# LiuZhu-CV/PAIF

Hardware: AMD Instinct MI355X
Metric: fused image-pairs/sec at 480x640 bs=8 per GPU (fusion-net forward) (higher is better)
Workload: dtype f16 (IEEE fp16 maps and conv weights, one fp16 MFMA per product, f32 accumulate; stems, guided filter and the last map fp32)

## Files before the change

include/paif_hip.h:

```cpp
#ifndef PAIF_HIP_H
#define PAIF_HIP_H

#include <stddef.h>
#include <stdint.h>

#ifdef __cplusplus
extern "C" {
#endif

#define PAIF_ABI_VERSION 1
#define PAIF_EINVAL (-1)
#define PAIF_ENOSUP (-2)

typedef void* paif_stream_t;

int paif_version(void);
const char* paif_last_error(void);
int paif_device_cus(void);


int paif_rgb2ycrcb_fwd(const float* rgb, float* ycc, int B, int H, int W, paif_stream_t stream);

int paif_ycrcb2rgb_fwd(const float* ycc, float* rgb, int B, int H, int W, paif_stream_t stream);

// ... 62 lines not shown
  float* cpool;
} paif_conv_desc;
#define PAIF_ST_F32 0
#define PAIF_ST_BF16 1
#define PAIF_ST_F32_BF16 2
#define PAIF_ST_F16 3
#define PAIF_ST_F16_F32 4
#define PAIF_CONV_F32 0
#define PAIF_CONV_BF16X3 1
#define PAIF_CONV_BF16 2
#define PAIF_CONV_F16 4
#define PAIF_CONV_F16X2 5
#define PAIF_CONV_F16X3 6
#define PAIF_CONV_BF16X6 3

int paif_dwconv_fwd_bf16(const float* x, const float* w, float* out, int k, int dil, int in_relu, int B, int H, int W,
                         paif_stream_t stream);
int paif_channel_pool2_fwd_bf16(const float* ir, const float* vis, float* comp, int B, int H, int W, paif_stream_t stream);
int paif_spa_blend_fwd_bf16(const float* comp, const float* w, const float* ir, const float* vis, float* agg, int B, int H, int W,
                            paif_stream_t stream);
int paif_eca_finish_fwd_bf16(const float* o, const float* r, const float* pool_partial, const float* w1d, int k,
                             const float* prelu, float* gate, float* out, int B, int H, int W, paif_stream_t stream);
int paif_tail_fwd_bf16(const float* x, const float* w, const float* prelu, float* fused, int B, int H, int W, paif_stream_t stream);
int paif_add_fwd_bf16(const float* a, const float* b, float* out, size_t n, paif_stream_t stream);
int paif_cast_storage_fwd(const float* src, float* dst, size_t n, int mode, paif_stream_t stream);
int paif_dwconv_fwd_f16(const float* x, const float* w, float* out, int k, int dil, int in_relu, int B, int H, int W,
                        paif_stream_t stream);
int paif_channel_pool2_fwd_f16(const float* ir, const float* vis, float* comp, int B, int H, int W, paif_stream_t stream);
int paif_spa_blend_fwd_f16(const float* comp, const float* w, const float* ir, const float* vis, float* agg, int B, int H, int W,
                           paif_stream_t stream);
int paif_eca_finish_fwd_f16(const float* o, const float* r, const float* pool_partial, const float* w1d, int k,
                            const float* prelu, float* gate, float* out, int B, int H, int W, paif_stream_t stream);
int paif_tail_fwd_f16(const float* x, const float* w, const float* prelu, float* fused, int B, int H, int W, paif_stream_t stream);
int paif_add_fwd_f16(const float* a, const float* b, float* out, size_t n, paif_stream_t stream);

int paif_conv2d_blocks(int B, int H, int W);
int paif_conv2d_fwd(const paif_conv_desc* d, int B, int H, int W, paif_stream_t stream);
int paif_conv2d_can_cpool(const paif_conv_desc* d, int B, int H, int W);
int paif_channel_pool1_fwd(const float* x, float* comp_off, int B, int H, int W, paif_stream_t stream);
int paif_channel_pool1_fwd_bf16(const float* x, float* comp_off, int B, int H, int W, paif_stream_t stream);
int paif_channel_pool1_fwd_f16(const float* x, float* comp_off, int B, int H, int W, paif_stream_t stream);
int paif_conv2d_is_persistent(const paif_conv_desc* d, int B, int H, int W);
int paif_conv2d_kernel_name(const paif_conv_desc* d, int B, int H, int W, char* buf, int buflen);
size_t paif_conv_wpk_floats(int nsrc, int cin, int kh);
int paif_pack_conv_weight(const float* w, float* wpk, int cout, int nsrc, int cin, int kh, paif_stream_t stream);
int paif_pack_conv_weight_bf16x3(const float* w, float* wpk, int cout, int nsrc, int kh, paif_stream_t stream);
int paif_pack_conv_weight_f16x2(const float* w, float* wpk, int cout, int nsrc, int kh, paif_stream_t stream);
int paif_pack_conv_weight_bf16x6(const float* w, float* wpk, int cout, int nsrc, int kh, paif_stream_t stream);
int paif_compose_dw_pw_weight(const float* dw, const float* pw, float* out, int cout, int cin, int kh, paif_stream_t stream);
int paif_compose_pw_conv_weight(const float* pw, const float* w, float* out, int cout, int cmid, int cin, int kh, paif_stream_t stream);

size_t paif_rdb_fused_wpk_floats(void);
int paif_rdb_fused_pack(const float* w1, const float* w2, const float* w3, float* wpk, int f16, paif_stream_t stream);
int paif_rdb_fused_fwd(const float* x, const float* wpk, const float* prelu, float alpha, const float* res0, const float* res1, float* out,
                       float* cpool, int f16, int reverse_tiles, int B, int H, int W, paif_stream_t stream);

int paif_stem_out_pack_floats(void);
int paif_stem_out_pack(const float* w1, const float* w2, float* wpk, paif_stream_t stream);
int paif_stem_out_fwd_bf16(const float* x, const float* wpk, const float* prelu, float* fused, int B, int H, int W, paif_stream_t stream);
int paif_stem_out_fwd_f32(const float* x, const float* wpk, const float* prelu, float* fused, int B, int H, int W, paif_stream_t stream);
int paif_stem_out_fwd_guard(const float* x, int f32in, const float* wpk, const float* prelu, float* fused, unsigned* flag, int B, int H, int W,
                            paif_stream_t stream);
int paif_pack_decomp1x1_weight_bf16x6(const float* w, float* wpk, paif_stream_t stream);
int paif_pack_decomp1x1_weight_bf16x3(const float* w, float* wpk, paif_stream_t stream);
int paif_pack_decomp1x1_hf_weight_f16x2(const float* w, float* wpk, paif_stream_t stream);
int paif_pack_decomp1x1_weight(const float* w, float* wpk, paif_stream_t stream);
// ... 260 lines not shown
```

paif_amd/_lib.py:

```python
import ctypes
import os
from ctypes import POINTER, Structure, c_char_p, c_float, c_int, c_size_t, c_ulonglong, c_void_p

HERE = os.path.dirname(os.path.abspath(__file__))
LIB_PATH = os.environ.get("PAIF_LIB") or os.path.join(HERE, "lib", "libpaif_hip.so")

F = c_void_p


class ConvDesc(Structure):

    _fields_ = [
        ("src", F * 3), ("nsrc", c_int), ("cin", c_int), ("wpk", F), ("kh", c_int), ("dil", c_int),
        ("in_act", c_int), ("in_prelu", F), ("scale", F), ("shift", F), ("act", c_int), ("prelu", F),
        ("alpha", c_float), ("res", F * 3), ("out", F), ("cout", c_int), ("pool_partial", F),
        ("precision", c_int), ("aux_out", F), ("in_aux", F), ("in_scale", F), ("in_alpha", c_float), ("epi_aux", F),
        ("epi_dact", c_int), ("reverse_tiles", c_int), ("storage", c_int), ("cpool", F),
    ]


SIGNATURES = {
    "paif_version": (c_int, []),
    "paif_last_error": (c_char_p, []),
    "paif_device_cus": (c_int, []),
# ... 81 lines not shown
    "paif_layernorm_fwd": (c_int, [F, F, F, F, c_int, c_int, c_float, F]),
    "paif_im2col_fwd": (c_int, [F, F, c_int, c_int, c_int, c_int, c_int, c_int, c_int, c_int, F]),
    "paif_pack_conv_gemm_weight": (c_int, [F, F, c_int, c_int, c_int, c_int, F]),
    "paif_dwconv3_bias_gelu_fwd": (c_int, [F, F, F, F, c_int, c_int, c_int, c_int, F]),
    "paif_sr_attention_fwd": (c_int, [F, F, F, F, c_int, c_int, c_int, c_int, c_int, F]),
    "paif_sr_attention_bf16x3_fwd": (c_int, [F, F, F, F, c_int, c_int, c_int, c_int, c_int, F]),
    "paif_sr_attention_split_fwd": (c_int, [F, F, F, F, c_int, c_int, c_int, c_int, c_int, c_int, F]),
    "paif_resize_bilinear_into_fwd": (c_int, [F, F, c_int, c_int, c_int, c_int, c_int, c_int, c_int, c_int, F]),
    "paif_nhwc_to_nchw_fwd": (c_int, [F, F, c_int, c_int, c_int, F]),
    "paif_nchw_to_nhwc_fwd": (c_int, [F, F, c_int, c_int, c_int, F]),
    "paif_nchw_to_nhwc_pad_fwd": (c_int, [F, F, c_int, c_int, c_int, c_int, F]),
    "paif_gemm_masked_fwd": (c_int, [F, c_int, F, F, F, F, F, c_int, F, c_int, F, c_int, c_int, c_int, c_int, c_int, F]),
    "paif_transpose_pad_fwd": (c_int, [F, F, c_int, c_int, c_int, F]),
    "paif_layernorm_bwd_input": (c_int, [F, F, F, F, F, c_int, c_int, c_float, F]),
    "paif_dwconv3_bias_gelu_bwd_input": (c_int, [F, F, F, F, F, F, c_int, c_int, c_int, c_int, F]),
    "paif_col2im_fwd": (c_int, [F, F, c_int, c_int, c_int, c_int, c_int, c_int, c_int, c_int, F]),
    "paif_resize_bilinear_adjoint_fwd": (c_int, [F, F, c_int, c_int, c_int, c_int, c_int, c_int, c_int, c_int, F]),
    "paif_sr_attention_bwd_chunks": (c_int, [c_int, c_int, c_int]),
    "paif_sr_attention_bwd_input": (c_int, [F, F, F, F, F, F, F, F, F, c_int, c_int, c_int, c_int, c_int, F]),
    "paif_sr_attention_bwd_input_p": (c_int, [F, F, F, F, F, F, F, F, F, c_int, c_int, c_int, c_int, c_int, c_int, F]),
    "paif_upsample_ce_blocks": (c_int, [c_int, c_int, c_int]),
    "paif_upsample_ce_fwd": (c_int, [F, F, F, F, c_int, c_int, c_int, c_int, c_int, c_int, c_int, F]),
    "paif_dwconv_fwd_bf16": (c_int, [F, F, F, c_int, c_int, c_int, c_int, c_int, c_int, F]),
    "paif_channel_pool2_fwd_bf16": (c_int, [F, F, F, c_int, c_int, c_int, F]),
    "paif_spa_blend_fwd_bf16": (c_int, [F, F, F, F, F, c_int, c_int, c_int, F]),
    "paif_eca_finish_fwd_bf16": (c_int, [F, F, F, F, c_int, F, F, F, c_int, c_int, c_int, F]),
    "paif_tail_fwd_bf16": (c_int, [F, F, F, F, c_int, c_int, c_int, F]),
    "paif_add_fwd_bf16": (c_int, [F, F, F, c_size_t, F]),
    "paif_dwconv_fwd_f16": (c_int, [F, F, F, c_int, c_int, c_int, c_int, c_int, c_int, F]),
    "paif_channel_pool2_fwd_f16": (c_int, [F, F, F, c_int, c_int, c_int, F]),
    "paif_spa_blend_fwd_f16": (c_int, [F, F, F, F, F, c_int, c_int, c_int, F]),
    "paif_eca_finish_fwd_f16": (c_int, [F, F, F, F, c_int, F, F, F, c_int, c_int, c_int, F]),
    "paif_tail_fwd_f16": (c_int, [F, F, F, F, c_int, c_int, c_int, F]),
    "paif_add_fwd_f16": (c_int, [F, F, F, c_size_t, F]),
    "paif_cast_storage_fwd": (c_int, [F, F, c_size_t, c_int, F]),
    "paif_attack_loss_blocks": (c_int, [c_int, c_int, c_int]),
    "paif_attack_loss_fwd": (c_int, [F, F, F, F, c_int, c_float, c_float, c_int, c_int, c_int, c_int, c_int, c_int, c_int, F]),
    "paif_attack_loss_bwd": (c_int, [F, F, F, F, c_int, c_float, c_float, c_float, c_int, c_int, c_int, c_int, c_int, c_int, c_int, c_int, F]),
    "paif_conv_weight_dgrad": (c_int, [F, F, c_int, c_int, c_int, c_int, c_int, F]),
    "paif_fold_decomp1x1_weight": (c_int, [F, F, F]),
    "paif_tail_bwd_input": (c_int, [F, F, F, F, F, F, c_int, c_int, c_int, F]),
    "paif_stem_bwd_input": (c_int, [F, F, F, F, F, c_int, c_int, c_int, F]),
    "paif_dwconv_bwd_input": (c_int, [F, F, F, F, F, c_int, c_int, c_int, c_int, c_int, F]),
    "paif_eca_bwd_blocks": (c_int, [c_int, c_int]),
    "paif_eca_bwd_input": (c_int, [F, F, F, F, F, c_int, F, F, F, F, F, c_int, c_int, c_int, F]),
    "paif_spa_blend_bwd_input": (c_int, [F, F, F, F, F, F, F, F, F, F, c_int, c_int, c_int, F]),
    "paif_guided_filter_bwd_input": (c_int, [F, F, F, F, c_float, c_float, F, F, F, F, F, F, c_int, c_int, c_int, F]),
    "paif_guided_filter_bwd_input_mc": (c_int, [F, F, F, F, F, F, F, F, F, F, c_int, c_int, c_int, F]),
    "paif_upsample_argmax_fwd": (c_int, [F, F, c_int, c_int, c_int, c_int, c_int, c_int, F]),
    "paif_confusion_matrix_accum": (c_int, [F, F, F, c_size_t, c_int, F]),
    "paif_spa1_fwd": (c_int, [F, F, F, c_int, F, F, F, F, F, c_int, c_int, c_int, F]),
    "paif_spa1_bwd_input": (c_int, [F, F, F, F, F, c_int, F, F, F, F, c_int, c_int, c_int, F]),
    "paif_glue_bwd_blocks": (c_int, [c_int, c_int, c_int]),
    "paif_glue_bwd_input": (c_int, [F, F, F, F, F, F, F, F, c_int, c_int, c_int, F]),
    "paif_plane_minmax_blocks": (c_int, [c_size_t]),
    "paif_plane_clamp_minmax_fwd": (c_int, [F, F, F, F, c_size_t, F]),
    "paif_plane_clamp_minmax_bwd_input": (c_int, [F, F, F, F, F, c_size_t, F]),
    "paif_channel_sum_chunks_fwd": (c_int, [F, F, c_int, c_int, c_int, c_int, F]),
    "paif_rgb2ycrcb_bwd_input": (c_int, [F, F, F, c_int, c_int, c_int, F]),
    "paif_pgd_step": (c_int, [F, F, F, c_float, c_float, c_size_t, F]),
    "paif_axpy": (c_int, [F, F, c_float, c_size_t, F]),
    "paif_upsample_ce_bwd": (c_int, [F, F, F, F, c_int, c_int, c_int, c_int, c_int, c_int, c_int, c_int, F]),
    "paif_head_sum_fwd": (c_int, [F, F, F, F, POINTER(c_int), F, F, F, c_int, c_int, F]),
    "paif_relu_mask_scale_fwd": (c_int, [F, F, F, F, c_size_t, c_int, F]),
    "paif_u8_to_planes_fwd": (c_int, [F, F, c_int, c_int, c_int, F]),
    "paif_u8_to_i64_fwd": (c_int, [F, F, c_size_t, F]),
# ... 71 lines not shown
```

paif_amd/csrc/fusion_kernels.hip:

```cpp
#include <stdarg.h>

#include "paif_common.h"

namespace paif {
static thread_local char g_err[256] = "";
void set_error(const char* fmt, ...) {
  va_list ap;
  va_start(ap, fmt);
  vsnprintf(g_err, sizeof(g_err), fmt, ap);
  va_end(ap);
}
}

namespace {

constexpr int MAXGRID = 256 * 8;

inline int grid_for(size_t work_items, int per_block) {
  size_t g = (work_items + per_block - 1) / per_block;
  if (g > (size_t)MAXGRID) g = MAXGRID;
  if (g < 1) g = 1;
  return (int)g;
}

__global__ void rgb2ycrcb_kernel(const float* __restrict__ rgb, float* __restrict__ ycc, int B, size_t HW) {
  const size_t total = (size_t)B * HW;
  for (size_t i = (size_t)blockIdx.x * blockDim.x + threadIdx.x; i < total; i += (size_t)gridDim.x * blockDim.x) {
    const size_t b = i / HW, px = i - b * HW;
    const float* s = rgb + b * 3 * HW + px;
    const float R = s[0], G = s[HW], Bl = s[2 * HW];
    const float Y = __fadd_rn(__fadd_rn(__fmul_rn(0.299f, R), __fmul_rn(0.587f, G)), __fmul_rn(0.114f, Bl));
    const float Cr = __fadd_rn(__fmul_rn(__fsub_rn(R, Y), 0.713f), 0.5f);
    const float Cb = __fadd_rn(__fmul_rn(__fsub_rn(Bl, Y), 0.564f), 0.5f);
    float* d = ycc + b * 3 * HW + px;
// ... 857 lines not shown
}
int paif_channel_pool1_fwd(const float* x, float* comp_off, int B, int H, int W, paif_stream_t stream) { return channel_pool1_launch(x, comp_off, B, H, W, 0, stream); }
int paif_channel_pool1_fwd_bf16(const float* x, float* comp_off, int B, int H, int W, paif_stream_t stream) { return channel_pool1_launch(x, comp_off, B, H, W, 1, stream); }
int paif_channel_pool1_fwd_f16(const float* x, float* comp_off, int B, int H, int W, paif_stream_t stream) { return channel_pool1_launch(x, comp_off, B, H, W, 2, stream); }

int paif_dwconv_fwd_bf16(const float* x, const float* w, float* out, int k, int dil, int in_relu, int B, int H, int W, paif_stream_t stream) {
  return dwconv16<1>(x, w, out, k, dil, in_relu, B, H, W, stream);
}
int paif_dwconv_fwd_f16(const float* x, const float* w, float* out, int k, int dil, int in_relu, int B, int H, int W, paif_stream_t stream) {
  return dwconv16<2>(x, w, out, k, dil, in_relu, B, H, W, stream);
}
int paif_channel_pool2_fwd_bf16(const float* ir, const float* vis, float* comp, int B, int H, int W, paif_stream_t stream) {
  return channel_pool2_16<1>(ir, vis, comp, B, H, W, stream);
}
int paif_channel_pool2_fwd_f16(const float* ir, const float* vis, float* comp, int B, int H, int W, paif_stream_t stream) {
  return channel_pool2_16<2>(ir, vis, comp, B, H, W, stream);
}
int paif_spa_blend_fwd_bf16(const float* comp, const float* w, const float* ir, const float* vis, float* agg, int B, int H, int W,
                            paif_stream_t stream) {
  return spa_blend16<1>(comp, w, ir, vis, agg, B, H, W, stream);
}
int paif_spa_blend_fwd_f16(const float* comp, const float* w, const float* ir, const float* vis, float* agg, int B, int H, int W,
                           paif_stream_t stream) {
  return spa_blend16<2>(comp, w, ir, vis, agg, B, H, W, stream);
}
int paif_eca_finish_fwd_bf16(const float* o, const float* r, const float* pool_partial, const float* w1d, int k, const float* prelu,
                             float* gate, float* out, int B, int H, int W, paif_stream_t stream) {
  return eca_finish16<1>(o, r, pool_partial, w1d, k, prelu, gate, out, B, H, W, stream);
}
int paif_eca_finish_fwd_f16(const float* o, const float* r, const float* pool_partial, const float* w1d, int k, const float* prelu,
                            float* gate, float* out, int B, int H, int W, paif_stream_t stream) {
  return eca_finish16<2>(o, r, pool_partial, w1d, k, prelu, gate, out, B, H, W, stream);
}
int paif_tail_fwd_bf16(const float* x, const float* w, const float* prelu, float* fused, int B, int H, int W, paif_stream_t stream) {
  return tail16<1>(x, w, prelu, fused, B, H, W, stream);
}
int paif_tail_fwd_f16(const float* x, const float* w, const float* prelu, float* fused, int B, int H, int W, paif_stream_t stream) {
  return tail16<2>(x, w, prelu, fused, B, H, W, stream);
}
int paif_add_fwd_bf16(const float* a, const float* b, float* out, size_t n, paif_stream_t stream) { return add16<1>(a, b, out, n, stream); }
int paif_add_fwd_f16(const float* a, const float* b, float* out, size_t n, paif_stream_t stream) { return add16<2>(a, b, out, n, stream); }

int paif_cast_storage_fwd(const float* src, float* dst, size_t n, int mode, paif_stream_t stream) {
  PAIF_REQUIRE(src && dst && n % 4 == 0, PAIF_EINVAL, "cast_storage: null pointer or n %% 4 != 0");
  PAIF_REQUIRE(mode >= 0 && mode <= 3, PAIF_EINVAL, "cast_storage: mode=%d", mode);
  if (n == 0) return 0;
  const dim3 g(grid_for(n / 4, 256)), blk(256);
  hipStream_t st = paif::as_stream(stream);
  switch (mode) {
    case 0: hipLaunchKernelGGL((cast_storage_kernel<1, 0>), g, blk, 0, st, src, dst, n / 4); break;
    case 1: hipLaunchKernelGGL((cast_storage_kernel<0, 1>), g, blk, 0, st, src, dst, n / 4); break;
    case 2: hipLaunchKernelGGL((cast_storage_kernel<0, 2>), g, blk, 0, st, src, dst, n / 4); break;
    default: hipLaunchKernelGGL((cast_storage_kernel<2, 0>), g, blk, 0, st, src, dst, n / 4); break;
  }
  PAIF_LAUNCH_CHECK("cast_storage");
  return 0;
}

int paif_minmax_blocks(int B, int H, int W) {
  const size_t total = (size_t)B * H * W;
  return (int)((total + MM_BLOCK_PIX - 1) / MM_BLOCK_PIX);
}

int paif_recompose_clamp_fwd(const float* fused, const float* ycc, float* rgb_out, float* minmax_partial, int B, int H,
                             int W, paif_stream_t stream) {
  PAIF_REQUIRE(fused && ycc && rgb_out && minmax_partial && B > 0 && H > 0 && W > 0, PAIF_EINVAL,
// ... 21 lines not shown
```

paif_amd/operations_m.py:

```python
import torch
import torch.nn as nn

from . import ops


class _NeverCalled:
    def forward(self, *a, **k):
        raise RuntimeError("%s is a parameter holder; the HIP path must be used" % type(self).__name__)


class Conv2dParams(_NeverCalled, nn.Conv2d):
    pass


class Conv1dParams(_NeverCalled, nn.Conv1d):
    pass


class BatchNormParams(_NeverCalled, nn.BatchNorm2d):
    pass


class PReLUParams(_NeverCalled, nn.PReLU):
    pass
# ... 435 lines not shown

class eca_layer(nn.Module):

    def __init__(self, channel, c_out, stride, k_size=3):
        super().__init__()
        self.k_size = k_size
        self.conv = Conv1dParams(1, 1, kernel_size=k_size, padding=(k_size - 1) // 2, bias=False)

    def forward(self, x):
        ops.require_no_grad(x)
        if x.shape[1] != 32:
            raise NotImplementedError("eca_layer: the HIP kernels are built for the 32-channel maps of the search space")
        with torch.no_grad():
            return ops.to_nchw_view(ops.eca_layer_fwd(ops.to_nhwc(x), self.conv.weight, self.k_size))


class ECABasicBlock(_HipOp):

    def __init__(self, inplanes, planes, kernel=3, dilation=1, stride=1, reduction=64, with_norm=False):
        super().__init__()
        if with_norm:
            raise NotImplementedError("ECABasicBlock(with_norm=True) is never constructed by the reference")
        self.with_norm = with_norm
        self.k = kernel
        self.conv1 = conv3x3(inplanes, planes, stride)
        self.conv2 = BasicConv(inplanes, inplanes, kernel, relu=False)
        self.se = eca_layer(planes, planes, stride, k_size=kernel)
        self.relu = PReLUParams()

    def forward_nhwc(self, x, res=(), tape=None):
        a = self.relu.weight
        w1 = self._packs.get("w1", [self.conv1.weight], lambda: ops.pack_conv_weight(self.conv1.weight, 1, 32, 3))
        r = ops.conv2d([x], w1, 3, 1)
        o, partial = ops.conv2d([r], self.conv2.wpk(1, 32), self.k, 1, in_act=ops.ACT_PRELU, in_prelu=a, pool=True)
        if tape is None:
            out = ops.eca_finish(o, r, partial, self.se.conv.weight, self.k, a)
        else:
            out, u, gate = ops.eca_finish(o, r, partial, self.se.conv.weight, self.k, a, save=True)
            tape.append(dict(r=r, o=o, u=u, gate=gate, x=x, pool=partial) if ops.taping_wgrad() else dict(r=r, o=o, u=u, gate=gate))
        return self._add_res(out, res)

    bwd_takes_res = True

    def backward_nhwc(self, g, t, wgrad=False, res=()):
        a = self.relu.weight
        if not wgrad:
            d_o, d_r = ops.eca_bwd(g, t["u"], t["o"], t["gate"], self.se.conv.weight, self.k, a)
            d_r = ops.conv2d([d_o], self._dgrad_w("c2", self.conv2.conv.weight), self.k, 1, epi_dact=1, epi_aux=t["r"], prelu=a, res=(d_r,))
            return ops.conv2d([d_r], self._dgrad_w("c1", self.conv1.weight), 3, 1, res=tuple(res))
        B, H, W, _ = g.shape
        ds = ops.grad_of(a)
        if ds is not None:
            ops.prelu_bwd(g, t["u"], a, ds)
        d_o, d_r, dgate = ops.eca_bwd(g, t["u"], t["o"], t["gate"], self.se.conv.weight, self.k, a, want_partial=True)
        g1d = ops.grad_of(self.se.conv.weight)
        if g1d is not None:
            ops.eca_wgrad(t["pool"], dgate, t["gate"], self.k, g1d, B, H, W)
        gw2 = ops.grad_of(self.conv2.conv.weight)
        if gw2 is not None:
            ops.conv2d_wgrad([ops.affine_act_res(t["r"], None, None, ops.ACT_PRELU, a)], d_o, self.k, 1, out=gw2)
        tt = ops.conv2d([d_o], self._dgrad_w("c2", self.conv2.conv.weight), self.k, 1)
        d_r = ops.prelu_bwd(tt, t["r"], a, ds, add=d_r, want_dx=True)
        gw1 = ops.grad_of(self.conv1.weight)
        if gw1 is not None:
            ops.conv2d_wgrad([t["x"]], d_r, 3, 1, out=gw1)
        return ops.conv2d([d_r], self._dgrad_w("c1", self.conv1.weight), 3, 1, res=tuple(res))


class Spatial_BasicBlock(_HipOp):

    def __init__(self, inplanes, planes, kernel=3, dilation=1, stride=1, reduction=64, with_norm=False):
        super().__init__()
# ... 94 lines not shown
```

paif_amd/ops.py:

```python
import ctypes
import weakref
import os

import torch

from . import _lib

ACT_NONE, ACT_PRELU, ACT_RELU = 0, 1, 2
ACT_GELU = 1

def _env_switch(name, default="1"):
    v = os.environ.get(name, default)
    if v not in ("0", "1", "gemm"):
        raise ValueError("%s=%r: expected 0, 1 or gemm" % (name, v))
    return {"0": False, "1": True, "gemm": "gemm"}[v]


GEMM_PRECISIONS = ("f32", "bf16x3", "auto", "bf16x6", "auto6", "f16x3", "auto6h")


def _env_gemm_precision():
    v = os.environ.get("PAIF_GEMM_PRECISION", "auto")
    if v not in GEMM_PRECISIONS:
        raise ValueError("PAIF_GEMM_PRECISION=%r: expected one of %s" % (v, GEMM_PRECISIONS))
# ... 802 lines not shown
    return comp


def spa_blend(comp, w, ir, vis, want_scale=False):
    B, H, W, _ = ir.shape
    agg = torch.empty_like(ir)
    if ir.dtype in H16:
        assert not want_scale and vis.dtype == ir.dtype
        fn = lib().paif_spa_blend_fwd_f16 if ir.dtype == torch.float16 else lib().paif_spa_blend_fwd_bf16
        _lib.check(fn(_p(comp), _p(w.detach().contiguous()), _pa(ir), _pa(vis), _pa(agg), B, H, W, _stream()), "spa_blend")
        return agg
    scale = torch.empty((B, H, W), device=ir.device, dtype=torch.float32) if want_scale else None
    _lib.check(lib().paif_spa_blend_fwd(_p(comp), _p(w.detach().contiguous()), _p(ir), _p(vis), _p(agg), _p(scale), B, H, W, _stream()),
               "spa_blend")
    return (agg, scale) if want_scale else agg


def eca_finish(o, r, partial, w1d, k, prelu, save=False):
    B, H, W, _ = o.shape
    out = torch.empty_like(o)
    gate = torch.empty((B, 32), device=o.device, dtype=torch.float32)
    if o.dtype in H16:
        assert not save and r.dtype == o.dtype
        fn = lib().paif_eca_finish_fwd_f16 if o.dtype == torch.float16 else lib().paif_eca_finish_fwd_bf16
        _lib.check(fn(_pa(o), _pa(r), _p(partial), _p(w1d.detach().contiguous()), k, _p(prelu), _p(gate), _pa(out),
                                                  B, H, W, _stream()), "eca_finish")
        return out
    u = torch.empty_like(o) if save else None
    _lib.check(lib().paif_eca_finish_fwd(_p(o), _p(r), _p(partial), _p(w1d.detach().contiguous()), k, _p(prelu), _p(gate), _p(out),
                                         _p(u), B, H, W, _stream()), "eca_finish")
    return (out, u, gate) if save else out


def eca_layer_fwd(x, w1d, k):
    B, H, W, C = x.shape
    assert C == 32 and x.dtype == torch.float32
    L = lib()
    chunks = L.paif_conv2d_blocks(1, H, W)
    partial = torch.empty((B, chunks, 32), device=x.device, dtype=torch.float32)
    _lib.check(L.paif_channel_sum_chunks_fwd(_p(x), _p(partial), chunks, B, H, W, _stream()), "channel_sum_chunks")
    one = torch.ones(1, device=x.device, dtype=torch.float32)
    return eca_finish(x, torch.zeros_like(x), partial, w1d, k, one)


def eca_bwd(dout, u, o, gate, w1d, k, prelu, want_partial=False):
    B, H, W, _ = o.shape
    L = lib()
    partial = torch.empty((B, L.paif_eca_bwd_blocks(H, W), 32), device=o.device, dtype=torch.float32)
    coef = torch.empty((B, 32), device=o.device, dtype=torch.float32)
    d_o, d_r = torch.empty_like(o), torch.empty_like(o)
    _lib.check(L.paif_eca_bwd_input(_p(dout), _p(u), _p(o), _p(gate), _p(w1d.detach().contiguous()), k, _p(prelu), _p(partial), _p(coef),
                                    _p(d_o), _p(d_r), B, H, W, _stream()), "eca_bwd")
    return (d_o, d_r, partial) if want_partial else (d_o, d_r)


def spa_blend_bwd(dagg, w, ir, vis, s, add_ir=None, add_vis=None, want_dpre=False):
    B, H, W, _ = ir.shape
    dpre = torch.empty((B, H, W), device=ir.device, dtype=torch.float32)
    d_ir, d_vis = torch.empty_like(ir), torch.empty_like(vis)
    _lib.check(lib().paif_spa_blend_bwd_input(_p(dagg), _p(w.detach().contiguous()), _p(ir), _p(vis), _p(s), _p(add_ir), _p(add_vis),
                                              _p(dpre), _p(d_ir), _p(d_vis), B, H, W, _stream()), "spa_blend_bwd")
    return (d_ir, d_vis, dpre) if want_dpre else (d_ir, d_vis)


def dwconv_bwd(dt, w, k, dil, aux=None, add=None):
    B, H, W, _ = dt.shape
# ... 1050 lines not shown
```

Before: 2609.

## Fuse ECA conv2, pooling and gating into row-streaming fp16 MFMA kernels

Adds a row-streaming 3x3 conv kernel that DMAs input rows straight into LDS, applies the input PReLU in place, and runs fp16 MFMA. In a pool pass it writes only per-tile channel sums instead of the conv output map. A second pass recomputes the conv and applies the ECA gate, residual and PReLU before writing the final map. This removes the write and re-read of the intermediate conv output and the separate eca_finish pass, at the cost of computing the conv twice. It is enabled by default through a size rule and is used only in inference when no tape is recorded.

```diff
diff --git a/include/paif_hip.h b/include/paif_hip.h
--- a/include/paif_hip.h
+++ b/include/paif_hip.h
@@ -118,6 +118,10 @@
 int paif_eca_finish_fwd_f16(const float* o, const float* r, const float* pool_partial, const float* w1d, int k,
                             const float* prelu, float* gate, float* out, int B, int H, int W, paif_stream_t stream);
 int paif_tail_fwd_f16(const float* x, const float* w, const float* prelu, float* fused, int B, int H, int W, paif_stream_t stream);
+int paif_eca_conv2_gated_fits(int B, int H, int W);
+int paif_eca_conv2_gated_fwd_f16(const float* r, const float* wpk, const float* in_prelu, float* pool_partial, const float* w1d, int k,
+                                 const float* prelu, float* gate, float* out, int B, int H, int W, paif_stream_t stream);
+int paif_eca_conv2_staged_f16(const float* r, const float* wpk, const float* in_prelu, float* out, int B, int H, int W, paif_stream_t stream);
 int paif_add_fwd_f16(const float* a, const float* b, float* out, size_t n, paif_stream_t stream);
 
 int paif_conv2d_blocks(int B, int H, int W);
diff --git a/paif_amd/_lib.py b/paif_amd/_lib.py
--- a/paif_amd/_lib.py
+++ b/paif_amd/_lib.py
@@ -137,6 +137,9 @@
     "paif_spa_blend_fwd_f16": (c_int, [F, F, F, F, F, c_int, c_int, c_int, F]),
     "paif_eca_finish_fwd_f16": (c_int, [F, F, F, F, c_int, F, F, F, c_int, c_int, c_int, F]),
     "paif_tail_fwd_f16": (c_int, [F, F, F, F, c_int, c_int, c_int, F]),
+    "paif_eca_conv2_gated_fits": (c_int, [c_int, c_int, c_int]),
+    "paif_eca_conv2_gated_fwd_f16": (c_int, [F, F, F, F, F, c_int, F, F, F, c_int, c_int, c_int, F]),
+    "paif_eca_conv2_staged_f16": (c_int, [F, F, F, F, c_int, c_int, c_int, F]),
     "paif_add_fwd_f16": (c_int, [F, F, F, c_size_t, F]),
     "paif_cast_storage_fwd": (c_int, [F, F, c_size_t, c_int, F]),
     "paif_attack_loss_blocks": (c_int, [c_int, c_int, c_int]),
diff --git a/paif_amd/csrc/conv_eca_rows.h b/paif_amd/csrc/conv_eca_rows.h
--- /dev/null
+++ b/paif_amd/csrc/conv_eca_rows.h
@@ -0,0 +1,24 @@
+#pragma once
+#include <hip/hip_runtime.h>
+
+namespace paif_eca_rows {
+
+struct Args {
+  const void* r;
+  const void* wpk;
+  const float* in_prelu;
+  const float* prelu;
+  const float* gate;
+  float* partial;
+  void* out;
+  int B, H, W;
+};
+
+enum Mode { POOL = 0, GATED = 1, STAGED = 2 };
+
+bool fits(int B, int H, int W);
+bool by_size_rule(int B, int H, int W);
+int env_switch();
+int launch(Mode m, const Args& a, hipStream_t st);
+
+}
diff --git a/paif_amd/csrc/conv_eca_rows.hip b/paif_amd/csrc/conv_eca_rows.hip
--- /dev/null
+++ b/paif_amd/csrc/conv_eca_rows.hip
@@ -0,0 +1,408 @@
+#include <stdint.h>
+#include <stdlib.h>
+
+#include <type_traits>
+
+#include "conv_eca_rows.h"
+#include "paif_common.h"
+
+namespace paif_eca_rows {
+namespace {
+
+typedef float f32x16 __attribute__((ext_vector_type(16)));
+typedef unsigned u32x4 __attribute__((ext_vector_type(4)));
+
+constexpr int RW = 32;
+constexpr int RWH = RW + 2;
+constexpr int TR = 8;
+constexpr int DPS = 3;
+constexpr int SLOT = DPS * 1024;
+constexpr int NSLOT = 5, PF = NSLOT - 3;
+constexpr int PARK = 32 * 32 * 4;
+constexpr int WAVE_LDS = NSLOT * SLOT + PARK;
+constexpr int WAVES = 4;
+constexpr int LDS_BYTES = WAVES * WAVE_LDS;
+constexpr int MAX_WAVES = 2048;
+constexpr int MIN_RUN = 2;
+constexpr int N_ROW = PF * DPS;
+static_assert(2 * LDS_BYTES <= 160 * 1024, "two workgroups per CU do not fit LDS");
+static_assert(RWH * 4 <= DPS * 64, "DMA instructions do not cover the row piece");
+constexpr unsigned RSRC_W3 = 0x00020000u;
+constexpr unsigned OOB = 0x80000000u;
+
+#ifndef ER_LD_AUX_POOL
+#define ER_LD_AUX_POOL 0
+#endif
+#ifndef ER_LD_AUX_GATED
+#define ER_LD_AUX_GATED 2
+#endif
+#ifndef ER_ST_AUX
+#define ER_ST_AUX 0
+#endif
+#define ER_VMWAIT(n) asm volatile("s_waitcnt vmcnt(%0)" ::"n"(n) : "memory")
+#define ER_RD128(dst, addr, off) asm volatile("ds_read_b128 %0, %1 offset:%2" : "=v"(dst) : "v"(addr), "n"(off) : "memory")
+#define ER_WR32(addr, val, off) asm volatile("ds_write_b32 %0, %1 offset:%2" ::"v"(addr), "v"(val), "n"(off) : "memory")
+#define ER_WR128(addr, val, off) asm volatile("ds_write_b128 %0, %1 offset:%2" ::"v"(addr), "v"(val), "n"(off) : "memory")
+
+template <int AUX>
+__device__ __forceinline__ void dma16(__amdgpu_buffer_rsrc_t rsrc, unsigned voff, unsigned lds_off) {
+  __builtin_amdgcn_raw_ptr_buffer_load_lds(rsrc, (__attribute__((address_space(3))) void*)(uintptr_t)lds_off, 16, voff, 0, 0, AUX);
+}
+
+__device__ __forceinline__ unsigned prelu_h2(unsigned x, float slope) {
+  typedef float f32x2 __attribute__((ext_vector_type(2)));
+  const f32x2 f = __builtin_convertvector(__builtin_bit_cast(paif::f16x2_t, x), f32x2) * slope;
+  const unsigned y = __builtin_bit_cast(unsigned, __builtin_convertvector(f, paif::f16x2_t));
+  unsigned t, m, r;
+  asm("v_pk_sub_u16 %0, %1, %2 clamp" : "=v"(t) : "v"(x), "v"(0x00010001u));
+  asm("v_pk_ashrrev_i16 %0, %1, %2" : "=v"(m) : "v"(0x000f000fu), "v"(t));
+  asm("v_bfi_b32 %0, %1, %2, %3" : "=v"(r) : "v"(m), "v"(y), "v"(x));
+  return r;
+}
+__device__ __forceinline__ u32x4 prelu_h8(u32x4 v, float slope) {
+  const unsigned a = v.x, b = v.y, c = v.z, d = v.w;
+  const u32x4 o = {prelu_h2(a, slope), prelu_h2(b, slope), prelu_h2(c, slope), prelu_h2(d, slope)};
+  return o;
+}
+
+template <int MODE>
+__global__ __launch_bounds__(WAVES * 64, 2) void eca_conv2_rows(Args a, int total, int SX, int TY, int run) {
+  constexpr int LD_AUX = MODE == POOL ? ER_LD_AUX_POOL : ER_LD_AUX_GATED;
+  __shared__ __attribute__((aligned(16))) unsigned char smem[LDS_BYTES];
+  asm volatile("" ::"v"((unsigned)(uintptr_t)(__attribute__((address_space(3))) unsigned char*)smem) : "memory");
+
+  const int tid = threadIdx.x, l = tid & 63;
+  const int w = __builtin_amdgcn_readfirstlane(tid >> 6);
+  const int p = l & 31, hh = l >> 5;
+  const int gw = blockIdx.x * WAVES + w;
+  int pos = gw * run;
+  const int end = min(total, pos + run);
+  if (pos >= end) return;
+  const int H = a.H, W = a.W;
+
+  const int map_bytes = a.B * H * W * 64;
+  const __amdgpu_buffer_rsrc_t rs_src = __builtin_amdgcn_make_buffer_rsrc(const_cast<void*>(a.r), 0, map_bytes, RSRC_W3);
+  const __amdgpu_buffer_rsrc_t rs_out = __builtin_amdgcn_make_buffer_rsrc(MODE == POOL ? (void*)a.partial : a.out, 0,
+                                                                          MODE == POOL ? a.B * TY * SX * 128 : map_bytes, RSRC_W3);
+
+  u32x4 bw[9][2];
+  {
+    const __amdgpu_buffer_rsrc_t rs_w = __builtin_amdgcn_make_buffer_rsrc(const_cast<void*>(a.wpk), 0, 9 * 2 * 2 * 1024, RSRC_W3);
+#pragma unroll
+    for (int tap = 0; tap < 9; ++tap)
+#pragma unroll
+      for (int ks = 0; ks < 2; ++ks) bw[tap][ks] = __builtin_amdgcn_raw_buffer_load_b128(rs_w, (unsigned)l * 16u, ((tap * 2 + ks) * 2) * 1024, 0);
+#pragma unroll
+    for (int tap = 0; tap < 9; ++tap) asm volatile("" : "+v"(bw[tap][0]), "+v"(bw[tap][1]));
+  }
+  float in_slope = *a.in_prelu;
+  float slope = MODE == GATED ? *a.prelu : 0.f;
+  asm volatile("" : "+v"(in_slope), "+v"(slope));
+
+  int d_col[DPS];
+  unsigned d_rel[DPS];
+#pragma unroll
+  for (int i = 0; i < DPS; ++i) {
+    const int n = 64 * i + l, c = n >> 2;
+    d_col[i] = c;
+    d_rel[i] = (unsigned)(c * 64 + (((n & 3) ^ ((c >> 2) & 3)) * 16));
+  }
+  const unsigned lds_w = (unsigned)(w * WAVE_LDS);
+  unsigned a_rd[3][2];
+#pragma unroll
+  for (int dx = 0; dx < 3; ++dx)
+#pragma unroll
+    for (int ks = 0; ks < 2; ++ks) {
+      const int c = p + dx;
+      a_rd[dx][ks] = lds_w + (unsigned)(c * 64 + (((2 * ks + hh) ^ ((c >> 2) & 3)) * 16));
+    }
+  const unsigned a_rw = lds_w + (unsigned)l * 16u;
+  const unsigned a_pw = lds_w + NSLOT * SLOT + (unsigned)((4 * hh * 32 + p) * 4);
+  const unsigned a_pr = lds_w + NSLOT * SLOT + (MODE == POOL ? (unsigned)((l >> 3) * 128 + (l & 7) * 16) : (unsigned)((l >> 2) * 128 + (l & 3) * 32));
+  unsigned a_st[2];
+#pragma unroll
+  for (int it = 0; it < 2; ++it) {
+    const int c = 16 * it + (l >> 2) + 1;
+    a_st[it] = lds_w + (unsigned)(c * 64 + (((l & 3) ^ ((c >> 2) & 3)) * 16));
+  }
+  const unsigned o_lane = (unsigned)l * 16u;
+
+  u32x4 rawr[2][2];
+  float ps[4] = {0.f, 0.f, 0.f, 0.f}, tot[4] = {0.f, 0.f, 0.f, 0.f};
+  f32x16 acc;
+
+  auto prelu_slot = [&](unsigned sb) {
+    u32x4 v0, v1, v2;
+    const unsigned ad = a_rw + sb;
+    ER_RD128(v0, ad, 0);
+    ER_RD128(v1, ad, 1024);
+    ER_RD128(v2, ad, 2048);
+    asm volatile("s_waitcnt lgkmcnt(0)" : "+v"(v0), "+v"(v1), "+v"(v2)::"memory");
+    v0 = prelu_h8(v0, in_slope);
+    v1 = prelu_h8(v1, in_slope);
+    v2 = prelu_h8(v2, in_slope);
+    ER_WR128(ad, v0, 0);
+    ER_WR128(ad, v1, 1024);
+    ER_WR128(ad, v2, 2048);
+  };
+
+  while (pos < end) {
+    const int q = pos / TY, ty0 = pos - q * TY;
+    const int k = min(TY - ty0, end - pos);
+    const int y0 = ty0 * TR;
+    const int n = min(H, (ty0 + k) * TR) - y0;
+    const int b = q / SX, sx = q - b * SX, x0 = sx * RW;
+    pos += k;
+    bool colok[DPS];
+#pragma unroll
+    for (int i = 0; i < DPS; ++i) colok[i] = d_col[i] < RWH && (unsigned)(x0 - 1 + d_col[i]) < (unsigned)W;
+    const bool xok0 = x0 + (l >> 2) < W, xok1 = x0 + 16 + (l >> 2) < W;
+    bool xokp[4];
+#pragma unroll
+    for (int it = 0; it < 4; ++it) xokp[it] = x0 + it * 8 + (l >> 3) < W;
+    float gt[8];
+    if constexpr (MODE == GATED) {
+      const __amdgpu_buffer_rsrc_t rs_g = __builtin_amdgcn_make_buffer_rsrc(const_cast<float*>(a.gate), 0, a.B * 128, RSRC_W3);
+      u32x4 g0 = __builtin_amdgcn_raw_buffer_load_b128(rs_g, (unsigned)(b * 128 + (l & 3) * 32), 0, 0);
+      u32x4 g1 = __builtin_amdgcn_raw_buffer_load_b128(rs_g, (unsigned)(b * 128 + (l & 3) * 32 + 16), 0, 0);
+      asm volatile("" : "+v"(g0), "+v"(g1));
+      gt[0] = __uint_as_float(g0.x); gt[1] = __uint_as_float(g0.y); gt[2] = __uint_as_float(g0.z); gt[3] = __uint_as_float(g0.w);
+      gt[4] = __uint_as_float(g1.x); gt[5] = __uint_as_float(g1.y); gt[6] = __uint_as_float(g1.z); gt[7] = __uint_as_float(g1.w);
+    }
+    auto issue_row = [&](int m, int slot) {
+      const int j = y0 - 1 + m;
+      const unsigned dead = (j >= 0 && j < H && m <= n + 1) ? 0u : OOB;
+      const unsigned rowb = (unsigned)((b * H + j) * W + x0 - 1) * 64u;
+#pragma unroll
+      for (int i = 0; i < DPS; ++i) dma16<LD_AUX>(rs_src, (colok[i] ? rowb + d_rel[i] : OOB) | dead, lds_w + (unsigned)(slot * SLOT + i * 1024));
+    };
+
+    int cur = 0;
+    auto step = [&](auto settag, int t) {
+      constexpr int SET = decltype(settag)::value;
+      const int s1 = cur + 1 >= NSLOT ? cur + 1 - NSLOT : cur + 1, s2 = cur + 2 >= NSLOT ? cur + 2 - NSLOT : cur + 2;
+      const int fill = cur == 0 ? NSLOT - 1 : cur - 1;
+      issue_row(t + 2 + PF, fill);
+      ER_VMWAIT(N_ROW);
+      const unsigned rb[3] = {(unsigned)(cur * SLOT), (unsigned)(s1 * SLOT), (unsigned)(s2 * SLOT)};
+      u32x4 n0, n1, n2;
+      const unsigned nad = a_rw + rb[2];
+      ER_RD128(n0, nad, 0);
+      ER_RD128(n1, nad, 1024);
+      ER_RD128(n2, nad, 2048);
+      if constexpr (MODE == GATED) {
+        const unsigned r0 = a_st[0] + rb[2], r1 = a_st[1] + rb[2];
+        ER_RD128(rawr[SET ^ 1][0], r0, 0);
+        ER_RD128(rawr[SET ^ 1][1], r1, 0);
+      }
+      u32x4 A[2][3][2];
+      auto read = [&](int buf, int dy) {
+#pragma unroll
+        for (int dx = 0; dx < 3; ++dx)
+#pragma unroll
+          for (int ks = 0; ks < 2; ++ks) {
+            const unsigned ad = a_rd[dx][ks] + rb[dy];
+            ER_RD128(A[buf][dx][ks], ad, 0);
+          }
+      };
+      auto mma = [&](auto dytag) {
+        constexpr int dy = decltype(dytag)::value, buf = dy & 1;
+#pragma unroll
+        for (int dx = 0; dx < 3; ++dx)
+#pragma unroll
+          for (int ks = 0; ks < 2; ++ks) {
+            if (dy == 0 && dx == 0 && ks == 0) {
+              const f32x16 z = {0.f, 0.f, 0.f, 0.f, 0.f, 0.f, 0.f, 0.f, 0.f, 0.f, 0.f, 0.f, 0.f, 0.f, 0.f, 0.f};
+              acc = paif::mfma16<2>(A[buf][dx][ks], bw[dy * 3 + dx][ks], z);
+            } else {
+              acc = paif::mfma16<2>(A[buf][dx][ks], bw[dy * 3 + dx][ks], acc);
+            }
+          }
+      };
+      read(0, 0);
+      read(1, 1);
+      if constexpr (MODE == GATED) {
+        asm volatile("s_waitcnt lgkmcnt(12)" : "+v"(n0), "+v"(n1), "+v"(n2), "+v"(rawr[SET ^ 1][0]), "+v"(rawr[SET ^ 1][1])::"memory");
+      } else {
+        asm volatile("s_waitcnt lgkmcnt(12)" : "+v"(n0), "+v"(n1), "+v"(n2)::"memory");
+      }
+      asm volatile("s_waitcnt lgkmcnt(6)"
+                   : "+v"(A[0][0][0]), "+v"(A[0][0][1]), "+v"(A[0][1][0]), "+v"(A[0][1][1]), "+v"(A[0][2][0]), "+v"(A[0][2][1])::"memory");
+      __builtin_amdgcn_sched_barrier(0);
+      mma(std::integral_constant<int, 0>{});
+      n0 = prelu_h8(n0, in_slope);
+      n1 = prelu_h8(n1, in_slope);
+      n2 = prelu_h8(n2, in_slope);
+      __builtin_amdgcn_sched_barrier(0);
+      ER_WR128(nad, n0, 0);
+      ER_WR128(nad, n1, 1024);
+      ER_WR128(nad, n2, 2048);
+      read(0, 2);
+      asm volatile("s_waitcnt lgkmcnt(9)"
+                   : "+v"(A[1][0][0]), "+v"(A[1][0][1]), "+v"(A[1][1][0]), "+v"(A[1][1][1]), "+v"(A[1][2][0]), "+v"(A[1][2][1])::"memory");
+      __builtin_amdgcn_sched_barrier(0);
+      mma(std::integral_constant<int, 1>{});
+      __builtin_amdgcn_sched_barrier(0);
+      asm volatile("s_waitcnt lgkmcnt(0)"
+                   : "+v"(A[0][0][0]), "+v"(A[0][0][1]), "+v"(A[0][1][0]), "+v"(A[0][1][1]), "+v"(A[0][2][0]), "+v"(A[0][2][1])::"memory");
+      __builtin_amdgcn_sched_barrier(0);
+      mma(std::integral_constant<int, 2>{});
+      __builtin_amdgcn_sched_barrier(0);
+
+      asm volatile("s_nop 15\n\ts_nop 7" ::: "memory");
+#pragma unroll
+      for (int r = 0; r < 16; ++r) {
+        const float v = acc[r];
+        ER_WR32(a_pw, v, ((r & 3) + 8 * (r >> 2)) * 128);
+      }
+      if constexpr (MODE == POOL) {
+        u32x4 tq[4];
+        ER_RD128(tq[0], a_pr, 0);
+        ER_RD128(tq[1], a_pr, 1024);
+        ER_RD128(tq[2], a_pr, 2048);
+        ER_RD128(tq[3], a_pr, 3072);
+        asm volatile("s_waitcnt lgkmcnt(0)" : "+v"(tq[0]), "+v"(tq[1]), "+v"(tq[2]), "+v"(tq[3])::"memory");
+        __builtin_amdgcn_sched_barrier(0);
+#pragma unroll
+        for (int it = 0; it < 4; ++it) {
+          const u32x4 tv = tq[it];
+          const float v0 = __uint_as_float(tv.x), v1 = __uint_as_float(tv.y), v2 = __uint_as_float(tv.z), v3 = __uint_as_float(tv.w);
+          ps[0] += xokp[it] ? v0 : 0.f;
+          ps[1] += xokp[it] ? v1 : 0.f;
+          ps[2] += xokp[it] ? v2 : 0.f;
+          ps[3] += xokp[it] ? v3 : 0.f;
+        }
+        const bool last = t == n - 1;
+        if (SET == 1 || last) {
+#pragma unroll
+          for (int c = 0; c < 4; ++c) {
+            float s = ps[c];
+            s += __shfl_xor(s, 8);
+            s += __shfl_xor(s, 16);
+            s += __shfl_xor(s, 32);
+            tot[c] += s;
+            ps[c] = 0.f;
+          }
+        }
+        if ((t & (TR - 1)) == TR - 1 || last) {
+          const int tile = (b * TY + ty0 + (t >> 3)) * SX + sx;
+          u32x4 od = {__float_as_uint(tot[0]), __float_as_uint(tot[1]), __float_as_uint(tot[2]), __float_as_uint(tot[3])};
+          __builtin_amdgcn_raw_buffer_store_b128(od, rs_out, l < 8 ? (unsigned)(tile * 128 + l * 16) : OOB, 0, 0);
+          asm volatile("s_nop 2" : "+v"(od));
+          tot[0] = tot[1] = tot[2] = tot[3] = 0.f;
+        }
+      } else {
+        u32x4 tq[2][2];
+        ER_RD128(tq[0][0], a_pr, 0);
+        ER_RD128(tq[0][1], a_pr, 16);
+        ER_RD128(tq[1][0], a_pr, 2048);
+        ER_RD128(tq[1][1], a_pr, 2048 + 16);
+        u32x4 sv[2];
+        if constexpr (MODE == STAGED) {
+          const unsigned c0 = a_st[0] + rb[1], c1 = a_st[1] + rb[1];
+          ER_RD128(sv[0], c0, 0);
+          ER_RD128(sv[1], c1, 0);
+          asm volatile("s_waitcnt lgkmcnt(0)" : "+v"(tq[0][0]), "+v"(tq[0][1]), "+v"(tq[1][0]), "+v"(tq[1][1]), "+v"(sv[0]), "+v"(sv[1])::"memory");
+        } else {
+          asm volatile("s_waitcnt lgkmcnt(0)" : "+v"(tq[0][0]), "+v"(tq[0][1]), "+v"(tq[1][0]), "+v"(tq[1][1])::"memory");
+        }
+        __builtin_amdgcn_sched_barrier(0);
+        const unsigned orow = (unsigned)((b * H + y0 + t) * W + x0) * 64u;
+#pragma unroll
+        for (int it = 0; it < 2; ++it) {
+          u32x4 od;
+          if constexpr (MODE == STAGED) {
+            od = sv[it];
+          } else {
+            const u32x4 t0 = tq[it][0], t1 = tq[it][1], rv = rawr[SET][it];
+            const float4 o0 = paif::f16x4_to_f32(paif::f32_to_f16x4(
+                make_float4(__uint_as_float(t0.x), __uint_as_float(t0.y), __uint_as_float(t0.z), __uint_as_float(t0.w))));
+            const float4 o1 = paif::f16x4_to_f32(paif::f32_to_f16x4(
+                make_float4(__uint_as_float(t1.x), __uint_as_float(t1.y), __uint_as_float(t1.z), __uint_as_float(t1.w))));
+            const float4 r0 = paif::f16x4_to_f32(make_uint2(rv.x, rv.y)), r1 = paif::f16x4_to_f32(make_uint2(rv.z, rv.w));
+            float4 u0, u1;
+            u0.x = __fadd_rn(__fmul_rn(o0.x, gt[0]), r0.x); u0.y = __fadd_rn(__fmul_rn(o0.y, gt[1]), r0.y);
+            u0.z = __fadd_rn(__fmul_rn(o0.z, gt[2]), r0.z); u0.w = __fadd_rn(__fmul_rn(o0.w, gt[3]), r0.w);
+            u1.x = __fadd_rn(__fmul_rn(o1.x, gt[4]), r1.x); u1.y = __fadd_rn(__fmul_rn(o1.y, gt[5]), r1.y);
+            u1.z = __fadd_rn(__fmul_rn(o1.z, gt[6]), r1.z); u1.w = __fadd_rn(__fmul_rn(o1.w, gt[7]), r1.w);
+            const uint2 h0 = paif::f32_to_f16x4(make_float4(paif::prelu_f(u0.x, slope), paif::prelu_f(u0.y, slope), paif::prelu_f(u0.z, slope),
+                                                            paif::prelu_f(u0.w, slope)));
+            const uint2 h1 = paif::f32_to_f16x4(make_float4(paif::prelu_f(u1.x, slope), paif::prelu_f(u1.y, slope), paif::prelu_f(u1.z, slope),
+                                                            paif::prelu_f(u1.w, slope)));
+            od = u32x4{h0.x, h0.y, h1.x, h1.y};
+          }
+          const bool ok = it ? xok1 : xok0;
+          __builtin_amdgcn_raw_buffer_store_b128(od, rs_out, ok ? orow + (unsigned)(it * 1024) + o_lane : OOB, 0, ER_ST_AUX);
+          asm volatile("s_nop 2" : "+v"(od));
+        }
+      }
+      __builtin_amdgcn_sched_barrier(0);
+      cur = s1;
+    };
+
+    static_assert(PF == 2 && NSLOT >= 4, "the prologue lists 2 + PF = 4 loads");
+    issue_row(0, 0);
+    issue_row(1, 1);
+    issue_row(2, 2);
+    issue_row(3, 3);
+    ER_VMWAIT(2 * DPS);
+    if constexpr (MODE == GATED) {
+      const unsigned r0 = a_st[0] + SLOT, r1 = a_st[1] + SLOT;
+      ER_RD128(rawr[0][0], r0, 0);
+      ER_RD128(rawr[0][1], r1, 0);
+      asm volatile("s_waitcnt lgkmcnt(0)" : "+v"(rawr[0][0]), "+v"(rawr[0][1])::"memory");
+    }
+    prelu_slot(0);
+    prelu_slot(SLOT);
+    for (int t = 0;; t += 2) {
+      step(std::integral_constant<int, 0>{}, t);
+      if (t + 1 >= n) break;
+      step(std::integral_constant<int, 1>{}, t + 1);
+      if (t + 2 >= n) break;
+    }
+    ER_VMWAIT(0);
+    asm volatile("s_waitcnt lgkmcnt(0)" ::: "memory");
+  }
+}
+
+template <int MODE>
+int launch_f(const Args& a, hipStream_t st, const char* what) {
+  const int SX = (a.W + RW - 1) / RW, TY = (a.H + TR - 1) / TR;
+  const int total = a.B * SX * TY;
+  const int per = (total + MAX_WAVES - 1) / MAX_WAVES;
+  const int run = per > MIN_RUN ? per : MIN_RUN;
+  const int waves = (total + run - 1) / run;
+  hipLaunchKernelGGL((eca_conv2_rows<MODE>), dim3((waves + WAVES - 1) / WAVES), dim3(WAVES * 64), 0, st, a, total, SX, TY, run);
+  hipError_t e = hipGetLastError();
+  if (e != hipSuccess) {
+    paif::set_error("%s: launch failed: %s", what, hipGetErrorString(e));
+    return (int)e;
+  }
+  return 0;
+}
+
+}
+
+int env_switch() {
+  const char* e = getenv("PAIF_ECA_ROWS");
+  if (!e || !e[0]) return -1;
+  return e[0] == '0' ? 0 : 1;
+}
+
+bool fits(int B, int H, int W) {
+  return B > 0 && H > 0 && W > 0 && (long long)B * H * W * 64 < (1ll << 31);
+}
+
+bool by_size_rule(int B, int H, int W) {
+  return fits(B, H, W) && H >= 64 && (long long)B * H * ((W + RW - 1) / RW) >= 32768;
+}
+
+int launch(Mode m, const Args& a, hipStream_t st) {
+  switch (m) {
+    case POOL: return launch_f<POOL>(a, st, "eca_conv2_rows(pool)");
+    case GATED: return launch_f<GATED>(a, st, "eca_conv2_rows(gated)");
+    default: return launch_f<STAGED>(a, st, "eca_conv2_rows(staged)");
+  }
+}
+
+}
diff --git a/paif_amd/csrc/fusion_kernels.hip b/paif_amd/csrc/fusion_kernels.hip
--- a/paif_amd/csrc/fusion_kernels.hip
+++ b/paif_amd/csrc/fusion_kernels.hip
@@ -1,5 +1,6 @@
 #include <stdarg.h>
 
+#include "conv_eca_rows.h"
 #include "paif_common.h"
 
 namespace paif {
@@ -923,6 +924,35 @@
                             float* gate, float* out, int B, int H, int W, paif_stream_t stream) {
   return eca_finish16<2>(o, r, pool_partial, w1d, k, prelu, gate, out, B, H, W, stream);
 }
+
+int paif_eca_conv2_gated_fits(int B, int H, int W) {
+  const int sw = paif_eca_rows::env_switch();
+  if (sw == 0) return 0;
+  return (sw == 1 ? paif_eca_rows::fits(B, H, W) : paif_eca_rows::by_size_rule(B, H, W)) ? 1 : 0;
+}
+int paif_eca_conv2_gated_fwd_f16(const float* r, const float* wpk, const float* in_prelu, float* pool_partial, const float* w1d, int k,
+                                 const float* prelu, float* gate, float* out, int B, int H, int W, paif_stream_t stream) {
+  PAIF_REQUIRE(r && wpk && in_prelu && pool_partial && w1d && prelu && gate && out && B > 0 && H > 0 && W > 0, PAIF_EINVAL,
+               "eca_conv2_gated: bad arguments");
+  PAIF_REQUIRE(k >= 1 && k <= 9 && (k & 1), PAIF_ENOSUP, "eca_conv2_gated: k=%d", k);
+  PAIF_REQUIRE(paif_eca_rows::fits(B, H, W), PAIF_ENOSUP, "eca_conv2_gated: %d x %d x %d x 32 fp16 does not fit 32-bit byte offsets", B, H, W);
+  hipStream_t st = paif::as_stream(stream);
+  paif_eca_rows::Args a = {};
+  a.r = r; a.wpk = wpk; a.in_prelu = in_prelu; a.prelu = prelu; a.gate = gate; a.partial = pool_partial; a.out = out;
+  a.B = B; a.H = H; a.W = W;
+  int e = paif_eca_rows::launch(paif_eca_rows::POOL, a, st);
+  if (e) return e;
+  hipLaunchKernelGGL(eca_scale_kernel, dim3(B), dim3(1024), 0, st, pool_partial, w1d, k, paif_conv2d_blocks(1, H, W), 1.0f / ((float)H * (float)W), gate);
+  PAIF_LAUNCH_CHECK("eca_scale");
+  return paif_eca_rows::launch(paif_eca_rows::GATED, a, st);
+}
+int paif_eca_conv2_staged_f16(const float* r, const float* wpk, const float* in_prelu, float* out, int B, int H, int W, paif_stream_t stream) {
+  PAIF_REQUIRE(r && wpk && in_prelu && out && paif_eca_rows::fits(B, H, W), PAIF_EINVAL, "eca_conv2_staged: bad arguments");
+  paif_eca_rows::Args a = {};
+  a.r = r; a.wpk = wpk; a.in_prelu = in_prelu; a.out = out;
+  a.B = B; a.H = H; a.W = W;
+  return paif_eca_rows::launch(paif_eca_rows::STAGED, a, paif::as_stream(stream));
+}
 int paif_tail_fwd_bf16(const float* x, const float* w, const float* prelu, float* fused, int B, int H, int W, paif_stream_t stream) {
   return tail16<1>(x, w, prelu, fused, B, H, W, stream);
 }
diff --git a/paif_amd/operations_m.py b/paif_amd/operations_m.py
--- a/paif_amd/operations_m.py
+++ b/paif_amd/operations_m.py
@@ -491,12 +491,11 @@
         a = self.relu.weight
         w1 = self._packs.get("w1", [self.conv1.weight], lambda: ops.pack_conv_weight(self.conv1.weight, 1, 32, 3))
         r = ops.conv2d([x], w1, 3, 1)
+        if tape is None:
+            return self._add_res(ops.eca_block_tail(r, self.conv2.wpk(1, 32), self.k, self.se.conv.weight, a), res)
         o, partial = ops.conv2d([r], self.conv2.wpk(1, 32), self.k, 1, in_act=ops.ACT_PRELU, in_prelu=a, pool=True)
-        if tape is None:
-            out = ops.eca_finish(o, r, partial, self.se.conv.weight, self.k, a)
-        else:
-            out, u, gate = ops.eca_finish(o, r, partial, self.se.conv.weight, self.k, a, save=True)
-            tape.append(dict(r=r, o=o, u=u, gate=gate, x=x, pool=partial) if ops.taping_wgrad() else dict(r=r, o=o, u=u, gate=gate))
+        out, u, gate = ops.eca_finish(o, r, partial, self.se.conv.weight, self.k, a, save=True)
+        tape.append(dict(r=r, o=o, u=u, gate=gate, x=x, pool=partial) if ops.taping_wgrad() else dict(r=r, o=o, u=u, gate=gate))
         return self._add_res(out, res)
 
     bwd_takes_res = True
diff --git a/paif_amd/ops.py b/paif_amd/ops.py
--- a/paif_amd/ops.py
+++ b/paif_amd/ops.py
@@ -858,6 +858,27 @@
     return (out, u, gate) if save else out
 
 
+ECA_ROWS_TAG = "eca_conv2_rows<0> + eca_scale_kernel + eca_conv2_rows<1>"
+
+
+def eca_block_tail(r, wpk, k, w1d, prelu):
+    B, H, W, C = r.shape
+    L = lib()
+    if r.dtype == torch.float16 and C == 32 and k == 3 and wpk.precision == "f16" and L.paif_eca_conv2_gated_fits(B, H, W):
+        out = torch.empty_like(r)
+        partial = torch.empty((L.paif_conv2d_blocks(B, H, W), 32), device=r.device, dtype=torch.float32)
+        gate = torch.empty((B, 32), device=r.device, dtype=torch.float32)
+        e0 = TIMER.start(ECA_ROWS_TAG) if TIMER is not None else None
+        _lib.check(L.paif_eca_conv2_gated_fwd_f16(_pa(r), _p(wpk.data), _p(prelu), _p(partial), _p(w1d.detach().contiguous()), k, _p(prelu),
+                                                  _p(gate), _pa(out), B, H, W, _stream()), "eca_conv2_gated")
+        if e0 is not None:
+            px = B * H * W
+            TIMER.stop(ECA_ROWS_TAG, e0, 2 * 2 * px * 9 * 32 * 32, px * 2 * 32 * 3)
+        return out
+    o, partial = conv2d([r], wpk, k, 1, in_act=ACT_PRELU, in_prelu=prelu, pool=True)
+    return eca_finish(o, r, partial, w1d, k, prelu)
+
+
 def eca_layer_fwd(x, w1d, k):
     B, H, W, C = x.shape
     assert C == 32 and x.dtype == torch.float32
```

After: 2640 (median of 6 runs). +1.2%, better.
